# nordmtr/quantpy

Hardware: AMD Instinct MI355X
Metric: state reconstructions/sec (3-qubit MLE) (higher is better)
Workload: dtype f64

## Files before the change

### quantpy_amd/csrc/qt_small.h

```cpp
#pragma once
#include <hip/hip_runtime.h>
#include <stdint.h>

#include <type_traits>

#include "qt_linesearch.h"

namespace qt {

#ifdef QT_PHASE_TIMING
__device__ long long* g_qt_prof = nullptr;
#define QT_PROF_ROW \
  ((size_t)(blockIdx.x + threadIdx.y * gridDim.x) * (blockDim.x >> 6) + (threadIdx.x >> 6))
#define QT_STAMP(slot)                                                                                   \
  do {                                                                                                   \
    if (g_qt_prof && (threadIdx.x & 63) == 0)                                                            \
      g_qt_prof[QT_PROF_ROW * 32 + (slot)] = (long long)__builtin_readcyclecounter();                    \
  } while (0)
#define QT_STAMP_VAL(slot, val)                                                                          \
  do {                                                                                                   \
    if (g_qt_prof && (threadIdx.x & 63) == 0)                                                            \
      g_qt_prof[QT_PROF_ROW * 32 + (slot)] = (val);                                                      \
  } while (0)
#else
#define QT_STAMP(slot) do {} while (0)
#define QT_STAMP_VAL(slot, val) do {} while (0)
#endif

struct alignas(16) cd {
  double re, im;
};
__device__ __forceinline__ cd cmul(cd a, cd b) { return {a.re * b.re - a.im * b.im, a.re * b.im + a.im * b.re}; }
__device__ __forceinline__ cd cmulc(cd a, cd b) {
  return {a.re * b.re + a.im * b.im, a.im * b.re - a.re * b.im};
}
__device__ __forceinline__ cd cadd(cd a, cd b) { return {a.re + b.re, a.im + b.im}; }
__device__ __forceinline__ cd hs_term(cd a, cd b) {
  return {__builtin_fma(a.re, b.re, -(a.im * b.im)), __builtin_fma(a.re, b.im, a.im * b.re)};
}
__device__ __forceinline__ cd cscale(cd a, double s) { return {a.re * s, a.im * s}; }

__device__ __forceinline__ void wave_sync() {
  __builtin_amdgcn_wave_barrier();
  asm volatile("" ::: "memory");
}

template <int CTRL, int ROW_MASK = 0xf>
__device__ __forceinline__ double dpp_f64(double v) {
  const long long b = __builtin_bit_cast(long long, v);
  const int lo = __builtin_amdgcn_update_dpp(0, (int)(b & 0xffffffffLL), CTRL, ROW_MASK, 0xf, ROW_MASK == 0xf);
  const int hi = __builtin_amdgcn_update_dpp(0, (int)(b >> 32), CTRL, ROW_MASK, 0xf, ROW_MASK == 0xf);
  return __builtin_bit_cast(double, ((long long)hi << 32) | (unsigned int)lo);
}
__device__ __forceinline__ double readlane_f64(double v, int lane) {
  const long long b = __builtin_bit_cast(long long, v);
  const int lo = __builtin_amdgcn_readlane((int)(b & 0xffffffffLL), lane);
  const int hi = __builtin_amdgcn_readlane((int)(b >> 32), lane);
  return __builtin_bit_cast(double, ((long long)hi << 32) | (unsigned int)lo);
}
__device__ __forceinline__ double nanmax(double a, double b) { return (b > a || b != b) ? b : a; }

template <int G>
__device__ __forceinline__ double gsum(double v) {
  v += dpp_f64<0xB1>(v);
  v += dpp_f64<0x4E>(v);
  if (G >= 8) v += dpp_f64<0x141>(v);
  if (G >= 16) v += dpp_f64<0x140>(v);
  if (G == 64) {
    v += dpp_f64<0x142, 0xA>(v);
    v += dpp_f64<0x143, 0xC>(v);
    v = readlane_f64(v, 63);
  }
  return v;
}
template <int G>
__device__ __forceinline__ bool group_any(bool pred) {
  const unsigned long long votes = __builtin_amdgcn_ballot_w64(pred);
  if (G == 64) return votes != 0ull;
  const int lane = threadIdx.x & 63;
  return (votes & (((1ull << (G & 63)) - 1ull) << (lane / G * G))) != 0ull;
}
__device__ __forceinline__ double max_f64(double a, double b) {
  double r;
  asm("v_max_f64 %0, %1, %2" : "=v"(r) : "v"(a), "v"(b));
  return r;
}
template <int G>
__device__ __forceinline__ double gmax(double v) {
  const bool nan = group_any<G>(v != v);
  v = max_f64(v, dpp_f64<0xB1>(v));
  v = max_f64(v, dpp_f64<0x4E>(v));
  if (G >= 8) v = max_f64(v, dpp_f64<0x141>(v));
  if (G >= 16) v = max_f64(v, dpp_f64<0x140>(v));
  if (G == 64) {
    v = max_f64(v, dpp_f64<0x142, 0xA>(v));
    v = max_f64(v, dpp_f64<0x143, 0xC>(v));
    v = readlane_f64(v, 63);
  }
  return nan ? __builtin_nan("") : v;
}

__device__ __forceinline__ double recip_nr(double x) {
  double r = __builtin_amdgcn_rcp(x);
  r = fma(r, fma(-x, r, 1.0), r);
  return fma(r, fma(-x, r, 1.0), r);
}
__device__ __forceinline__ bool log_is_regular(double x) { return x > 0.0 && x < 1.7e308; }
__device__ __forceinline__ double fast_log(double x) {
  if (!(x > 0.0) || !(x < 1.7e308)) return x == 0.0 ? -__builtin_huge_val() : (x > 0.0 ? x : __builtin_nan(""));
  double m = __builtin_amdgcn_frexp_mant(x);
  int e = __builtin_amdgcn_frexp_exp(x);
  const bool low = m < 0.70710678118654752440;
  m = low ? m + m : m;
  e = low ? e - 1 : e;
  const double num = m - 1.0, den = m + 1.0;
  const double r = recip_nr(den);
  double sq = num * r;
  sq = fma(r, fma(-sq, den, num), sq);
  const double z = sq * sq;
  const double z2 = z * z, z4 = z2 * z2, z8 = z4 * z4;
  const double q0 = fma(z, 1.0 / 5.0, 1.0 / 3.0), q1 = fma(z, 1.0 / 9.0, 1.0 / 7.0);
  const double q2 = fma(z, 1.0 / 13.0, 1.0 / 11.0), q3 = fma(z, 1.0 / 17.0, 1.0 / 15.0);
  const double q4 = fma(z, 1.0 / 21.0, 1.0 / 19.0);
  const double r0 = fma(z2, q1, q0), r1 = fma(z2, q3, q2);
  const double pl = fma(z8, q4, fma(z4, r1, r0));
  const double lm = fma(sq + sq, pl * z, sq + sq);
  const double ed = (double)e;
  return fma(ed, 6.93147180369123816490e-01, fma(ed, 1.90821492927058770002e-10, lm));
}

constexpr bool kLiftSingleNegative = true;

__device__ __forceinline__ double fast_rsqrt(double x) {
  double y = __builtin_amdgcn_rsq(x);
  double e = fma(-x * y, y, 1.0);
  y = fma(y * e, fma(e, 0.375, 0.5), y);
  e = fma(-x * y, y, 1.0);
  return fma(y * e, 0.5, y);
}

template <int UNR>
__device__ __forceinline__ void dot_block(const double* __restrict__ base, size_t stride, unsigned lane_off,
                                          const double* lds_vec, int m, double (&acc)[4]) {
  double av[UNR];
#pragma unroll
  for (int u = 0; u < UNR; ++u) av[u] = base[(size_t)(m + u) * stride + lane_off];
#pragma unroll
  for (int u = 0; u < UNR; ++u) acc[u & 3] = fma(av[u], lds_vec[m + u], acc[u & 3]);
  __builtin_amdgcn_sched_group_barrier(0x020, UNR, 0);
#pragma unroll
  for (int u = 0; u < UNR; u += 4) {
    __builtin_amdgcn_sched_group_barrier(0x100, 2, 0);
    __builtin_amdgcn_sched_group_barrier(0x002, 4, 0);
  }
}
template <int UNR>
__device__ __forceinline__ double dot_global(const double* __restrict__ base, size_t stride, unsigned lane_off,
                                             const double* lds_vec, int n) {
  double acc[4] = {0.0, 0.0, 0.0, 0.0};
  int m = 0;
  for (; m + UNR <= n; m += UNR) dot_block<UNR>(base, stride, lane_off, lds_vec, m, acc);
  if (UNR > 8 && m + 8 <= n) {
    dot_block<8>(base, stride, lane_off, lds_vec, m, acc);
    m += 8;
  }
  if (UNR > 4 && m + 4 <= n) {
    dot_block<4>(base, stride, lane_off, lds_vec, m, acc);
    m += 4;
  }
  for (; m < n; ++m) acc[0] = fma(base[(size_t)m * stride + lane_off], lds_vec[m], acc[0]);
  return (acc[0] + acc[1]) + (acc[2] + acc[3]);
}

__device__ __forceinline__ void rotation(double app, double aqq, cd apq, double& cs, cd& w) {
  const double ab2 = apq.re * apq.re + apq.im * apq.im;
  cs = 1.0;
  w = cd{0.0, 0.0};
  if (ab2 > 1e-300) {
    const double dl = 0.5 * (aqq - app);
    const double x = fma(dl, dl, ab2);
    double y = __builtin_amdgcn_rsq(x);
    y = fma(y * fma(-x * y, y, 1.0), 0.5, y);
    const double den = fabs(dl) + x * y;
    double z = __builtin_amdgcn_rcp(den);
    z = fma(z, fma(-den, z, 1.0), z);
    const double u = copysign(z, dl);
    cs = fast_rsqrt(fma(u * u, ab2, 1.0));
    const double cu = cs * u;
    w = cd{cu * apq.re, cu * apq.im};
  }
}


struct ProductView {
  const double* T;
  const double* P1T;
  const double* wrowR;
  const int* rmap;
  const int* rinv;
  const int* fwd;
  const int* bwd;
  int R1;
  int uniform;
  double wuni;
  int enabled;
  int pairedT, pairedP;
  double cT[12], cP[12];
  const int* last;
};

struct PovmView {
  const double* Aw;
  const double* AwT;
  const double* PinvT;
  int M;
  ProductView pr;
  double jtol2 = 1e-28;
  const double* Ns = nullptr;
  int S = 0, K = 0;
  double ns_tot = 0.0;
  int extra = 0;
};

struct SpecArgs {
  const void* image;
  const double* Ns;
  double ns_tot, wuni, jtol2;
  int M, extra;
  double cT[12], cP[12];
};
template <bool GENERIC>
struct MleArgs {
  using type = PovmView;
};
template <>
struct MleArgs<false> {
  using type = SpecArgs;
};

__device__ __forceinline__ bool shots_match(double t_s, double total, double n_s, double ns_tot) {
  const double a = t_s * ns_tot, b = n_s * total;
  return fabs(a - b) <= 2e-15 * fabs(b);
}

__device__ __forceinline__ const double* centre_of(const double* centres, int G, int g0, int b, int dd) {
  return G > 1 ? centres + (size_t)((unsigned)(g0 + b) % (unsigned)G) * dd : centres;
}

struct EstOut {
// ... 435 lines not shown
  __device__ __forceinline__ static bool seg_check(const double (&dv)[4], const bool (&valid)[4], double total,
                                                   const Prefetch& pf, double ns_tot) {
    bool bad = false;
#pragma unroll
    for (int q = 0; q < 4; ++q) bad |= valid[q] & !shots_match(segsum_c<KK>(dv[q]), total, pf.ns[q], ns_tot);
    return bad;
  }
  __device__ static bool load_freq(const Ctx& c, const int64_t* counts, const Prefetch* pf = nullptr) {
    double part = 0.0;
    double* raw = c.rbuf();
    double* fq = c.freq();
    bool bad = false;
    double total, inv;
    if (pf && pf->ok) {
      double dv[4];
      bool valid[4];
#pragma unroll
      for (int q = 0; q < 4; ++q) {
        const int m = c.l + q * G;
        valid[q] = m < c.M;
        dv[q] = valid[q] ? (double)pf->v[q] : 0.0;
        raw[valid[q] ? m : c.Mp] = dv[q];
        part += dv[q];
      }
      total = gsum<G>(part);
      inv = 1.0 / total;
      if (pf->seg) {
        switch (c.pv.K) {
          case 2: bad = seg_check<2>(dv, valid, total, *pf, c.pv.ns_tot); break;
          case 4: bad = seg_check<4>(dv, valid, total, *pf, c.pv.ns_tot); break;
          case 8: bad = seg_check<8>(dv, valid, total, *pf, c.pv.ns_tot); break;
          default: bad = seg_check<16>(dv, valid, total, *pf, c.pv.ns_tot); break;
        }
      }
      wave_sync();
#pragma unroll
      for (int q = 0; q < 4; ++q) {
        const int m = c.l + q * G, mc = m < c.M ? m : c.M - 1;
        fq[mc] = raw[c.prod() ? c.trmap[mc] : mc] * inv;
      }
    } else {
      for (int m = c.l; m < c.M; m += G) {
        const double v = (double)counts[m];
        raw[m] = v;
        part += v;
      }
      total = gsum<G>(part);
      inv = 1.0 / total;
      wave_sync();
      if (c.prod()) {
        for (int m = c.l; m < c.M; m += G) fq[m] = raw[c.trmap[m]] * inv;
      } else {
        for (int m = c.l; m < c.M; m += G) fq[m] = raw[m] * inv;
      }
    }
    if (c.pv.Ns && !(pf && pf->seg)) {
      const int K = c.pv.K;
      for (int s = c.l; s < c.pv.S; s += G) {
        double t = 0.0;
        for (int k = 0; k < K; ++k) t += raw[s * K + k];
        const double ns = (pf && s == c.l) ? pf->ns[0] : c.pv.Ns[s];
        bad |= !shots_match(t, total, ns, c.pv.ns_tot);
      }
    }
    const unsigned long long votes = __builtin_amdgcn_ballot_w64(bad);
    const int lane = threadIdx.x & 63;
    const unsigned long long mine = (G == 64) ? ~0ull : (((1ull << (G & 63)) - 1ull) << (lane / G * G));
    wave_sync();
    return (votes & mine) == 0ull;
  }

  __device__ __forceinline__ static void prefetch_counts(Prefetch& pf, const int64_t* counts, const SpecArgs& a) {
    const int l = (threadIdx.x & 63) % G, M = a.M, nch = image_chunks(M), t = threadIdx.x;
    const uint4* img = reinterpret_cast<const uint4*>(a.image);
    const int* rinv = reinterpret_cast<const int*>(img + nch);
    pf.img = img[t < nch ? t : nch - 1];
    if constexpr (NQ == 3) pf.mat = MakeMatTab<true, D>::type::v[l];
    pf.ok = pf.seg = true;
#pragma unroll
    for (int q = 0; q < 4; ++q) {
      const int m = l + q * G, mc = m < M ? m : M - 1;
      pf.v[q] = counts[mc];
      pf.ri[q] = rinv[mc];
      pf.ns[q] = a.Ns[mc >> NQ];
    }
  }
  template <bool VCOEF = false, bool TWIN = false, int LT>
  __device__ static void make_ctx(CtxSV<LT>& c, double* smem_block, const SpecArgs& a, const Prefetch& pf,
                                  [[maybe_unused]] int twin = 0) {
    static_assert(VCOEF == (LT == 2), "the one-wave-per-SIMD kernels keep coefficients and lane tables in vector registers");
    const int lane = threadIdx.x & 63, wave = threadIdx.x >> 6;
    c.l = lane % G;
    const int slot = wave * TPW + lane / G;
    c.i = c.l / d;
    c.j = c.l % d;
    c.e = c.i * LD + c.j;
    c.M = a.M;
    c.Mp = (a.M + 1) & ~1;
    c.a = a;
    if (!(TWIN && twin) && (int)threadIdx.x < image_chunks(a.M)) reinterpret_cast<uint4*>(smem_block)[threadIdx.x] = pf.img;
    c.tfwd = reinterpret_cast<const int*>(smem_block);
    c.ttab = smem_block + image_last_ints(a.M) / 2;
    c.ptab = c.ttab + 24;
    c.sm = smem_block + table_doubles(a.M, 6) + slot * (trial_doubles(a.M, 6) + a.extra);
    if (TWIN && twin) c.sm = smem_block + twin_offset(a.M, 6, a.extra) + slot * trial_doubles(a.M, 6);
    if (c.l == 0) c.sm[oVec + D] = 0.0;
    __syncthreads();
    int xm = 0, zm = 0, ny = 0;
#pragma unroll
    for (int b = 0; b < NQ; ++b) {
      const int dig = (c.l >> (2 * b)) & 3;
      xm |= (dig == 1 || dig == 2) << b;
      zm |= (dig >= 2) << b;
      ny += dig == 2;
    }
    c.xm = xm;
    c.zm = zm;
    c.ny = ny & 3;
    param_owner(c.l, c.pi, c.pj, c.pkind);
    const int tt = (c.i * (c.i - 1)) / 2 + c.j;
    c.src_re = c.i == c.j ? c.i : c.i > c.j ? d + tt : D;
    c.src_im = c.i > c.j ? d + T + tt : D;
    const int sx = (c.i & 1) | ((c.i & 2) << 1) | ((c.i & 4) << 2), sz = (c.j & 1) | ((c.j & 2) << 1) | ((c.j & 4) << 2);
    c.bslot = sx ^ (3 * sz);
    if constexpr (NQ == 3 && LT != 0) {
      c.mpack[0] = (uint32_t)pf.mat;
      c.mpack[1] = (uint32_t)(pf.mat >> 32);
      if constexpr (VCOEF) {
#pragma unroll
        for (int s = 0; s < d; ++s) {
          const uint32_t e = (c.mpack[s / 4] >> (8 * (s % 4))) & 0xffu;
          c.mterm[s] = c.sm + oVec + (e & 63u);
          c.msign[s] = (e & 0x80u) << 24;
        }
        c.bflip[0] = (uint32_t)lane << 31;
        c.bflip[1] = ((uint32_t)lane << 30) & 0x80000000u;
        c.bflip[2] = ((uint32_t)lane << 29) & 0x80000000u;
        c.bflip[3] = ((uint32_t)__popc(c.i & c.j) << 30) & 0x80000000u;
      }
    }
#pragma unroll
    for (int k = 0; k < 12; ++k) {
      c.kT[k] = VCOEF ? pin_vgpr(a.cT[k]) : a.cT[k];
      c.kP[k] = VCOEF ? pin_vgpr(a.cP[k]) : a.cP[k];
    }
  }
  template <int KK>
  __device__ __forceinline__ static double gsum_above(double v) {
    if (KK < 2) v += dpp_f64<0xB1>(v);
    if (KK < 4) v += dpp_f64<0x4E>(v);
    if (G >= 8 && KK < 8) v += dpp_f64<0x141>(v);
    if (G >= 16 && KK < 16) v += dpp_f64<0x140>(v);
    if (G == 64) {
      v += dpp_f64<0x142, 0xA>(v);
      v += dpp_f64<0x143, 0xC>(v);
      v = readlane_f64(v, 63);
    }
    return v;
  }
  template <int LT>
  __device__ static bool load_freq(const CtxSV<LT>& c, const Prefetch& pf) {
    double dv[4], st[4];
    bool valid[4];
#pragma unroll
    for (int q = 0; q < 4; ++q) {
      valid[q] = c.l + q * G < c.M;
      dv[q] = valid[q] ? (double)pf.v[q] : 0.0;
      st[q] = segsum_c<d>(dv[q]);
    }
    const double total = gsum_above<d>((st[0] + st[1]) + (st[2] + st[3]));
    const double inv = 1.0 / total;
    bool bad = false;
#pragma unroll
    for (int q = 0; q < 4; ++q) bad |= valid[q] & !shots_match(st[q], total, pf.ns[q], c.a.ns_tot);
    double* fq = c.freq();
    double* dummy = c.rbuf();
#pragma unroll
    for (int q = 0; q < 4; ++q) *(valid[q] ? fq + pf.ri[q] : dummy) = dv[q] * inv;
    const unsigned long long votes = __builtin_amdgcn_ballot_w64(bad);
    const int lane = threadIdx.x & 63;
    const unsigned long long mine = (G == 64) ? ~0ull : (((1ull << (G & 63)) - 1ull) << (lane / G * G));
    wave_sync();
    return (votes & mine) == 0ull;
  }

  __device__ __forceinline__ static int ipow(int b, int e) {
    int r = 1;
    for (int q = 0; q < e; ++q) r *= b;
    return r;
  }
  template <bool FWD, int R1C = 0>
  __device__ __forceinline__ static double stage_value(const double* tb, int R1, int ent, int stride, const double* in) {
    const int base = ent & 0xffff, sel = ent >> 16;
    if (FWD) {
      const double* row = tb + sel * 4;
      return fma(row[3], in[base + 3 * stride],
                 fma(row[2], in[base + 2 * stride], fma(row[1], in[base + stride], row[0] * in[base])));
    }
    double acc = 0.0;
    if (R1C > 0) {
      double tv[R1C > 0 ? R1C : 1], iv[R1C > 0 ? R1C : 1];
#pragma unroll
      for (int t = 0; t < R1C; ++t) {
        tv[t] = tb[t * 4 + sel];
        iv[t] = in[base + t * stride];
      }
#pragma unroll
      for (int t = 0; t < R1C; ++t) acc = fma(tv[t], iv[t], acc);
      return acc;
    }
    for (int t = 0; t < R1; ++t) acc = fma(tb[t * 4 + sel], in[base + t * stride], acc);
    return acc;
  }
  template <bool FWD, int R1C, class C>
  __device__ __forceinline__ static void stage_run(const C& c, const double* tb, const int* tab, int n_out, int stride,
                                                   const double* in, double* out) {
    const int R1 = c.R1();
    for (int o = c.l; o < n_out; o += 2 * G) {
      const int o2 = o + G;
      const bool two = o2 < n_out;
      const int e0 = tab[o], e1 = tab[two ? o2 : o];
      const double v0 = stage_value<FWD, R1C>(tb, R1, e0, stride, in);
      const double v1 = stage_value<FWD, R1C>(tb, R1, e1, stride, in);
      out[o] = v0;
      if (two) out[o2] = v1;
    }
  }
  template <bool FWD, class C>
  __device__ static void stage(const C& c, const double* tb, const int* tab, int n_out, int stride, const double* in,
                               double* out) {
    if (FWD) stage_run<true, 0>(c, tb, tab, n_out, stride, in, out);
    else if (c.R1() == 6) stage_run<false, 6>(c, tb, tab, n_out, stride, in, out);
    else if (c.R1() == 4) stage_run<false, 4>(c, tb, tab, n_out, stride, in, out);
    else stage_run<false, 0>(c, tb, tab, n_out, stride, in, out);
    wave_sync();
  }
  template <int R1C, class C>
  __device__ __forceinline__ static double stage_last(const C& c, const double* tb, const int* tab, const double* in) {
    return stage_value<false, R1C>(tb, c.R1(), tab[c.l], 1 << (2 * (NQ - 1)), in);
  }
  __device__ __forceinline__ static int paired_bases(int q) { return ipow(6, q - 1) << (2 * (NQ - q)); }
  template <class C>
  __device__ __forceinline__ static void paired_forward(const C& c, int q, const double* in, double* out) {
    const int lk = 2 * (NQ - q), Kq = 1 << lk;
    if (c.l < paired_bases(q)) {
      const int rpre = c.l >> lk, krest = c.l & (Kq - 1);
      const double* ib = in + ((rpre * 4) << lk) + krest;
      double* ob = out + ((rpre * 6) << lk) + krest;
      const double x0 = ib[0];
      const double xa[3] = {ib[Kq], ib[2 * Kq], ib[3 * Kq]};
#pragma unroll
      for (int r = 0; r < 6; ++r) ob[r * Kq] = fma(c.cT(2 * r + 1), xa[r >> 1], c.cT(2 * r) * x0);
    }
    wave_sync();
  }
  template <bool PINV, class C>
  __device__ __forceinline__ static void paired_backward(const C& c, int q, const double* in, double* out) {
    const int lk = 2 * (NQ - q), Kq = 1 << lk;
    if (c.l < paired_bases(q)) {
      const int rpre = c.l >> lk, krest = c.l & (Kq - 1);
      const double* ib = in + ((rpre * 6) << lk) + krest;
      double* ob = out + ((rpre * 4) << lk) + krest;
      double y[6], acc = 0.0;
#pragma unroll
      for (int t = 0; t < 6; ++t) y[t] = ib[t * Kq];
#pragma unroll
      for (int t = 0; t < 6; ++t) acc = fma(PINV ? c.cP(2 * t) : c.cT(2 * t), y[t], acc);
      ob[0] = acc;
#pragma unroll
      for (int a = 0; a < 3; ++a) {
        const double v0 = PINV ? c.cP(4 * a + 1) : c.cT(4 * a + 1);
        const double v1 = PINV ? c.cP(4 * a + 3) : c.cT(4 * a + 3);
        ob[(a + 1) * Kq] = fma(v1, y[2 * a + 1], v0 * y[2 * a]);
      }
    }
    wave_sync();
  }

  template <bool PINV, class C>
  __device__ static double prod_backward(const C& c, const double* yn) {
    const double* tb = PINV ? c.tabP() : c.tabT();
    const double* in = yn;
    double* bufs[2] = {c.bufB(), c.rbuf()};
    int which = 0;
    if (PINV ? c.pairedP() : c.pairedT()) {
#pragma unroll
      for (int q = NQ; q >= 2; --q) {
        paired_backward<PINV>(c, q, in, bufs[which]);
        in = bufs[which];
        which ^= 1;
      }
      const int lk = 2 * (NQ - 1);
      return stage_value<false, 6>(tb, 6, (c.l & ((1 << lk) - 1)) | (c.l >> lk) << 16, 1 << lk, in);
    }
    if constexpr (C::kGeneric) {
      const int R1 = c.R1();
      const int* tab = c.tbwd;
#pragma unroll
      for (int q = NQ; q >= 2; --q) {
        const int stride = 1 << (2 * (NQ - q));
        const int n_out = ipow(R1, q - 1) * 4 * stride;
        stage<false>(c, tb, tab, n_out, stride, in, bufs[which]);
        tab += n_out;
        in = bufs[which];
        which ^= 1;
      }
      if (R1 == 6) return stage_last<6>(c, tb, tab, in);
      if (R1 == 4) return stage_last<4>(c, tb, tab, in);
// ... 310 lines not shown
      if (!(mag > 1e-13)) neg = neg > 0 ? 99 : neg;
      const double safe = mag > 1e-300 ? mag : 1e-300;
      if (k + 1 < d) {
        const double inv = recip_nr(safe);
        const double sinv = pos ? -inv : inv;
        const cd ajs{ajk.re * sinv, ajk.im * sinv};
        const bool upd = i > k && j > k;
        const double nre = fma(aik.re, ajs.re, fma(aik.im, ajs.im, a.re));
        const double nim = fma(aik.im, ajs.re, fma(-aik.re, ajs.im, a.im));
        a.re = upd ? nre : a.re;
        a.im = upd ? nim : a.im;
        A[c.e] = a;
        wave_sync();
      }
    }
    {
      const double dj = A[j * LD + j].re;
      const double mj = fabs(dj);
      const double rs = fast_rsqrt(mj > 1e-300 ? mj : 1e-300);
      if (i >= j) lmine = (i == j) ? cd{dj * rs, 0.0} : cd{a.re * rs, a.im * rs};
    }
    ok = neg == 0;
    if (neg_out) *neg_out = neg;
    if (kneg_out) *kneg_out = kneg;
    if (SPEC && spec_inv) *spec_inv = b;
    L[c.e] = lmine;
    wave_sync();
    const cd e = L[c.pi * LD + c.pj];
    const double x = c.pkind == 2 ? e.im : e.re;
    wave_sync();
    return x;
  }

  struct HelperLink {
    enum : int { kPending = 0, kGo = 1, kAbort = 2, kClaimed = 3, kRevoked = 4 };
    enum : int { kNothing = 0, kLifted = 1, kRefused = 2 };
    static constexpr int kHelperPolls = 1 << 15, kWaitPolls = 1 << 14, kClaimedPolls = 1 << 16;
    double* base;
    int pending;
    __device__ __forceinline__ static constexpr int doubles() { return MAT + D + 3; }
    __device__ __forceinline__ cd* result() const { return reinterpret_cast<cd*>(base); }
    __device__ __forceinline__ double* x() const { return base + MAT; }
    __device__ __forceinline__ int* verdict() const { return reinterpret_cast<int*>(base + MAT + D); }
    __device__ __forceinline__ int* lifted() const { return verdict() + 1; }
    __device__ __forceinline__ int* done() const { return verdict() + 2; }
    __device__ __forceinline__ int* gone() const { return verdict() + 3; }
    __device__ __forceinline__ int* ok() const { return verdict() + 4; }
    __device__ __forceinline__ static void publish(int* w, int v) {
      wave_sync();
      if ((threadIdx.x & 63) == 0) __hip_atomic_store(w, v, __ATOMIC_RELEASE, __HIP_MEMORY_SCOPE_WORKGROUP);
    }
    __device__ __forceinline__ static int peek(const int* w) {
      return __builtin_amdgcn_readfirstlane(__hip_atomic_load(w, __ATOMIC_RELAXED, __HIP_MEMORY_SCOPE_WORKGROUP));
    }
    __device__ __forceinline__ static bool claim(int* w, int from, int to) {
      int won = 0;
      if ((threadIdx.x & 63) == 0) {
        int expect = from;
        won = __hip_atomic_compare_exchange_strong(w, &expect, to, __ATOMIC_ACQ_REL, __ATOMIC_RELAXED,
                                                   __HIP_MEMORY_SCOPE_WORKGROUP);
      }
      return __builtin_amdgcn_readfirstlane(won) != 0;
    }
    template <int SLEEP>
    __device__ __forceinline__ static int poll(const int* w, int idle, int polls) {
      int v = idle;
#pragma unroll 1
      for (int n = 0; n < polls; ++n) {
        v = peek(w);
        if (v != idle) break;
        __builtin_amdgcn_s_sleep(SLEEP);
      }
      return v;
    }
    __device__ __forceinline__ void reset() {
      pending = 0;
      if ((threadIdx.x & 63) == 0) {
        *verdict() = kPending;
        *lifted() = kNothing;
        *done() = 0;
        *gone() = 0;
      }
    }
    __device__ __forceinline__ void decide(bool go) const { publish(verdict(), go ? kGo : kAbort); }
    __device__ __forceinline__ int await_lift(int e, cd& proj) {
      int v = poll<1>(lifted(), kNothing, kWaitPolls);
      if (v == kNothing) {
        if (claim(verdict(), kGo, kRevoked)) return kNothing;
        v = poll<1>(lifted(), kNothing, kClaimedPolls);
        if (v == kNothing) return kNothing;
      }
      __builtin_amdgcn_fence(__ATOMIC_ACQUIRE, "workgroup");
      if (v == kLifted) {
        proj = result()[e];
        pending = 1;
      }
      return v;
    }
    __device__ __forceinline__ bool collect(int l, double& xl, int& okl) const {
      if (poll<1>(done(), 0, kClaimedPolls) == 0) return false;
      __builtin_amdgcn_fence(__ATOMIC_ACQUIRE, "workgroup");
      xl = x()[l];
      okl = *ok();
      return true;
    }
    __device__ __forceinline__ void await_gone() const {
      poll<1>(gone(), 0, kClaimedPolls);
      __builtin_amdgcn_fence(__ATOMIC_ACQUIRE, "workgroup");
    }
  };
  struct CtxH {
    int l, i, j, e, pi, pj, pkind;
    cd *image, *second, *factor;
    const int* verdict;
    __device__ __forceinline__ cd* A() const { return image; }
    __device__ __forceinline__ cd* Bm() const { return factor; }
    __device__ __forceinline__ cd* V() const { return second; }
    __device__ __forceinline__ int verdict_load() const {
      return __hip_atomic_load(verdict, __ATOMIC_RELAXED, __HIP_MEMORY_SCOPE_WORKGROUP);
    }
    __device__ __forceinline__ static bool abandoned(int v) {
      v = __builtin_amdgcn_readfirstlane(v);
      return v != HelperLink::kPending && v != HelperLink::kGo;
    }
  };
  struct LateX {
    bool got;
    double x;
    int ok;
  };
  template <class Base>
  struct WithHelper : Base {
    HelperLink* link;
    LateX* late;
    double* xtra;
    __device__ __forceinline__ double* extra() const { return xtra; }
    static constexpr bool kHelper = true;
  };
  __device__ __forceinline__ static void param_owner(int l, int& pi, int& pj, int& pkind) {
    const bool diag = l < d, imag = l >= d + T;
    const int t = l - d - (imag ? T : 0);
    int ii = 1;
#pragma unroll
    for (int k = 2; k < d; ++k) ii += t >= (k * (k - 1)) / 2;
    pkind = diag ? 0 : imag ? 2 : 1;
    pi = diag ? l : ii;
    pj = diag ? l : t - (ii * (ii - 1)) / 2;
  }
  template <class C>
  __device__ static bool twin_lift(const C& t, const HelperLink& k, cd lin, cd& proj) {
    static_assert(G == 64, "one trial per wavefront");
    CtxH c = side_ctx(t, k, t.Bm());
    proj = cd{0.0, 0.0};
    const bool lifted = __builtin_amdgcn_readfirstlane((int)lift_single_negative(c, lin, d - 1, 1e-15, proj, nullptr)) != 0;
    QT_STAMP(6);
    if (HelperLink::template poll<1>(k.verdict(), HelperLink::kPending, HelperLink::kHelperPolls) != HelperLink::kGo) return false;
    QT_STAMP(7);
    if (!HelperLink::claim(k.verdict(), HelperLink::kGo, HelperLink::kClaimed)) return false;
    if (!lifted) {
      HelperLink::publish(k.lifted(), HelperLink::kRefused);
      return false;
    }
    k.result()[c.e] = proj;
    HelperLink::publish(k.lifted(), HelperLink::kLifted);
    return true;
  }
  template <class C>
  __device__ static void sweep_for(const C& t, const HelperLink& k, cd proj, cd* L) {
    CtxH c = side_ctx(t, k, L);
    int ok2;
    const double x2 = cholesky_param(c, proj, ok2);
    k.x()[c.l] = x2;
    if (c.l == 0) *k.ok() = ok2;
    HelperLink::publish(k.done(), 1);
    QT_STAMP(7);
  }
  template <class C>
  __device__ __forceinline__ static CtxH side_ctx(const C& t, const HelperLink& k, cd* L) {
    CtxH c;
    c.l = t.l;
    c.i = t.i;
    c.j = t.j;
    c.e = t.e;
    c.pi = t.pi;
    c.pj = t.pj;
    c.pkind = t.pkind;
    c.image = t.A();
    c.second = t.V();
    c.factor = L;
    c.verdict = k.verdict();
    return c;
  }

  template <class C>
  __device__ static bool lift_single_negative(const C& c, cd r, int kneg, double eps, cd& out,
                                              const cd* inverse = nullptr) {
    static_assert(G == 64, "one trial per wavefront: the flags below are wave-uniform");
    cd* Ai = c.A();
    cd* Vi = c.V();
    const int i = c.i, j = c.j;
    if (i == j) r.im = 0.0;
    cd b = r;
    if (inverse) b = *inverse;
#pragma unroll 1
    for (int s = inverse ? d : 0; s < d; ++s) {
      const int p = s < kneg ? s : (s < d - 1 ? s + 1 : kneg);
      Ai[c.e] = b;
      const double piv = readlane_f64(b.re, p * d + p);
      wave_sync();
      const cd bip = Ai[i * LD + p], bpj = Ai[p * LD + j];
      wave_sync();
      double inv = __builtin_amdgcn_rcp(piv);
      inv = fma(inv, fma(-piv, inv, 1.0), inv);
      inv = fma(inv, fma(-piv, inv, 1.0), inv);
      const cd t{bpj.re * inv, bpj.im * inv};
      const cd e = cmul(bip, t);
      cd nb{b.re - e.re, b.im - e.im};
      if (j == p) nb = cd{-bip.re * inv, -bip.im * inv};
      if (i == p) nb = (j == p) ? cd{inv, 0.0} : t;
      b = nb;
    }
    QT_STAMP(4);
    b = cscale(b, fast_rsqrt(gsum<G>(b.re * b.re + b.im * b.im)));
    bool certified = false, done = false;
#pragma unroll 1
    for (int k = 1; k <= 7 && !done; ++k) {
      Ai[c.e] = b;
      wave_sync();
      [[maybe_unused]] const int verdict = c.verdict_load();
      cd n{0.0, 0.0}, n2{0.0, 0.0};
#pragma unroll
      for (int q = 0; q < d; q += 2) {
        const cd u = Ai[i * LD + q], v = Ai[j * LD + q];
        n.re = fma(u.re, v.re, fma(u.im, v.im, n.re));
        n.im = fma(u.im, v.re, fma(-u.re, v.im, n.im));
        if (q + 1 < d) {
          const cd u2 = Ai[i * LD + q + 1], v2 = Ai[j * LD + q + 1];
          n2.re = fma(u2.re, v2.re, fma(u2.im, v2.im, n2.re));
          n2.im = fma(u2.im, v2.re, fma(-u2.re, v2.im, n2.im));
        }
      }
      n = cadd(n, n2);
      wave_sync();
      if (c.abandoned(verdict)) return false;
      const double pur = gsum<G>(n.re * n.re + n.im * n.im);
      b = cscale(n, fast_rsqrt(pur));
      const double defect = 1.0 - pur;
      QT_STAMP_VAL(20, k);
#ifdef QT_PHASE_TIMING
      if (k <= 5) QT_STAMP(25 + k);
#endif
      if (certified) done = true;
      else if (defect < 1e-7) certified = true;
      else if (k == 3 && !(defect < 0.05)) return false;
    }
    QT_STAMP(5);
    if (!done) return false;
    if (i == j) b.im = 0.0;
    b = cscale(b, 1.0 / gsum<G>(i == j ? b.re : 0.0));
    const double lam = gsum<G>(r.re * b.re + r.im * b.im);
    if (!(lam < eps)) return false;
    Ai[c.e] = r;
    Vi[c.e] = b;
    wave_sync();
    cd q{-lam * b.re, -lam * b.im};
#pragma unroll
    for (int k = 0; k < d; ++k) {
      const cd u = Ai[i * LD + k], v = Vi[j * LD + k];
      q.re = fma(u.re, v.re, fma(u.im, v.im, q.re));
      q.im = fma(u.im, v.re, fma(-u.re, v.im, q.im));
    }
    wave_sync();
    const double res2 = gsum<G>(q.re * q.re + q.im * q.im);
    const double nrm2 = gsum<G>(r.re * r.re + r.im * r.im);
    if (!(res2 <= 1e-26 * nrm2)) return false;
    const double w = eps - lam;
    cd o{fma(w, b.re, r.re), fma(w, b.im, r.im)};
    const double tr = gsum<G>(i == j ? o.re : 0.0);
    out = cd{o.re / tr, o.im / tr};
    return true;
  }

  template <bool SPEC = false, class C>
  __device__ static cd make_feasible(const C& c, cd r, double* xl, int* ok_out, double* lscale_out = nullptr) {
    int ok, neg, kneg;
    cd spec_inv{0.0, 0.0};
    double x = cholesky_param<SPEC && G == 64>(c, r, ok, &neg, &kneg, &spec_inv);
    QT_STAMP(3);
    cd out{0.0, 0.0};
    double lscale = 1.0;
    auto pd_epilogue = [&]() {
      const double tr = gsum<G>(c.i == c.j ? r.re : 0.0);
      out = cd{r.re / tr, r.im / tr};
      const double rst = tr > 0.0 ? fast_rsqrt(tr) : 1.0 / sqrt(tr);
      x = x * rst;
      lscale = rst;
    };
    const bool all_pd = __all(ok);
    [[maybe_unused]] bool go = false;
    if constexpr (C::kHelper) {
      go = kLiftSingleNegative && !all_pd && __builtin_amdgcn_readfirstlane(neg) == 1 &&
           __builtin_amdgcn_readfirstlane(kneg) == d - 1;
      c.link->decide(go);
    }
    if (G < 64 || all_pd || (!xl && lscale_out)) pd_epilogue();
    if (!all_pd) {
      cd proj;
      bool lifted = false;
      [[maybe_unused]] bool refused = false;
      if constexpr (C::kHelper) {
        if (go) {
          const int came = c.link->await_lift(c.e, proj);
          QT_STAMP(31);
          if (came == HelperLink::kLifted) {
            QT_STAMP(6);
            if (lscale_out) *lscale_out = 1.0;
            return proj;
          }
          refused = came == HelperLink::kRefused;
        }
      }
      if constexpr (G == 64) {
        if (kLiftSingleNegative && !refused && __builtin_amdgcn_readfirstlane(neg) == 1) {
          const int kn = __builtin_amdgcn_readfirstlane(kneg);
          lifted = __builtin_amdgcn_readfirstlane(
                       (int)lift_single_negative(c, r, kn, 1e-15, proj, SPEC && kn == d - 1 ? &spec_inv : nullptr)) != 0;
        }
      }
      if (!lifted) proj = psd_project(c, r, 1e-15);
      QT_STAMP(6);
      int ok2 = 1;
      double x2 = xl ? cholesky_param(c, proj, ok2) : 0.0;
      if (lifted && xl && !__all(ok2 || ok)) {
        proj = psd_project(c, r, 1e-15);
        x2 = cholesky_param(c, proj, ok2);
      }
      QT_STAMP(7);
      if (xl) lscale = 1.0;
      if (!ok) {
        out = proj;
        x = x2;
        ok = ok2;
      }
    }
    if (xl) *xl = x;
    if (ok_out) *ok_out = ok;
    if (lscale_out) *lscale_out = lscale;
    return out;
  }

  template <class C>
  __device__ static cd build_llh(const C& c, double xl, double& tr) {
    double* vx = c.vec();
    cd* L = c.Bm();
    vx[c.l] = xl;
    tr = gsum<G>(xl * xl);
    wave_sync();
    const int i = c.i, j = c.j;
    L[c.e] = cd{vx[c.src_re], vx[c.src_im]};
    wave_sync();
    cd m{0.0, 0.0};
#pragma unroll
    for (int k = 0; k < d; ++k) {
      const cd u = L[i * LD + k], v = L[j * LD + k];
      m.re = fma(u.re, v.re, fma(u.im, v.im, m.re));
      m.im = fma(u.im, v.re, fma(-u.re, v.im, m.im));
    }
    return m;
  }

  struct StartPoint {
    cd rho;
    double lscale;
  };
  template <bool DEFER = false, class C, bool LATE = false>
  __device__ static void nll_grad(const C& c, double xl, double& f, double& gl, cd* rho_l = nullptr,
                                  bool want_grad = true, const StartPoint* start = nullptr, DeferredValue* dv = nullptr) {
    static_assert(!DEFER || !C::kGeneric, "the deferred value needs the compile-time row count of the specialised shape");
    double tr;
    QT_STAMP(11);
    cd m;
    if constexpr (LATE) {
      m = start->rho;
    } else if (start) {
      tr = gsum<G>(xl * xl);
      m = cd{start->rho.re * tr, start->rho.im * tr};
    } else {
      m = build_llh(c, xl, tr);
    }
    QT_STAMP(12);
    cd* A = c.A();
    const cd rho_e = start ? start->rho : cd{m.re / tr, m.im / tr};
    if (rho_l) *rho_l = rho_e;
    A[c.e] = rho_e;
    wave_sync();
    const double bl = bloch_of(c, A);
    QT_STAMP(13);
    double* vec = c.vec();
    vec[c.l] = bl;
    wave_sync();
    double fpart = 0.0;
    const double* fr = c.freq();
    double* rb = c.rbuf();
    double wl;
    if (c.prod()) {
      const int R1 = c.R1();
      const bool paired = c.pairedT() != 0;
      const int* tab = c.tfwd;
      const double* in = vec;
#pragma unroll
      for (int q = 1; q < NQ; ++q) {
        const int stride = 1 << (2 * (NQ - q));
        const int n_out = ipow(R1, q) * stride;
        double* out = ((NQ - 1 - q) & 1) ? rb : c.bufB();
        if (paired) {
          paired_forward(c, q, in, out);
        } else if constexpr (C::kGeneric) {
          stage<true>(c, c.tabT(), tab, n_out, stride, in, out);
          tab += n_out;
        }
        in = out;
      }
      QT_STAMP(14);
      if constexpr (DEFER) {
        stage_n_log<true, true, true>(c, tab, in, fr, rb, dv);
      } else if constexpr (!C::kGeneric) {
        fpart = stage_n_log<true, true>(c, tab, in, fr, rb);
      } else {
        if (!paired) fpart = stage_n_log<false, false>(c, tab, in, fr, rb);
        else if (c.uniform()) fpart = stage_n_log<true, true>(c, tab, in, fr, rb);
        else fpart = stage_n_log<true, false>(c, tab, in, fr, rb);
      }
      if constexpr (!DEFER) f = -gsum<G>(fpart);
      wave_sync();
      QT_STAMP(15);
      if (!want_grad) return;
      wl = prod_backward<false>(c, rb);
      QT_STAMP(16);
    } else if constexpr (C::kGeneric) {
      for (int m0 = 0; m0 < c.M; m0 += G) {
        const int mm = m0 + c.l;
        if (mm < c.M) {
          const double pe = row_dot(c, c.pv.AwT, mm, vec) * d + 1e-10;
          fpart += fr[mm] * fast_log(pe);
          rb[mm] = fr[mm] * recip_nr(pe);
// ... 754 lines not shown
```

Baseline: 110.7 million.

## Trim wavefront reductions, add diagonal trace reduction, unroll natural-order pivot elimination

Wave-level sum and max reductions drop the row masks on the final two DPP row-broadcast steps, since only lane 63 is read afterwards. A specialised gtrace reduction sums only the 8 diagonal lanes of the 8x8 matrix using one DPP shift and a few readlanes instead of a full tree, and it replaces every trace computation. The helper-side lift uses a compile-time natural pivot order with a fully unrolled elimination loop. The power-iteration loop folds its exit conditions into one branch and checks abandonment without an early return. The risks are subtle lane-index assumptions in gtrace (lane i*9 holds diagonal entry i for d=8) and a longer loop iteration when the work is abandoned.

```diff
diff --git a/quantpy_amd/csrc/qt_small.h b/quantpy_amd/csrc/qt_small.h
--- a/quantpy_amd/csrc/qt_small.h
+++ b/quantpy_amd/csrc/qt_small.h
@@ -67,11 +67,21 @@
   if (G >= 8) v += dpp_f64<0x141>(v);
   if (G >= 16) v += dpp_f64<0x140>(v);
   if (G == 64) {
-    v += dpp_f64<0x142, 0xA>(v);
-    v += dpp_f64<0x143, 0xC>(v);
+    v += dpp_f64<0x142>(v);
+    v += dpp_f64<0x143>(v);
     v = readlane_f64(v, 63);
   }
   return v;
+}
+template <int G>
+__device__ __forceinline__ double gtrace(bool diag, double x) {
+  double v = diag ? x : 0.0;
+  if (G != 64) return gsum<G>(v);
+  v += 0.0;
+  v += dpp_f64<0x119>(v);
+  const double hi = v + readlane_f64(v, 45);
+  const double lo = v + readlane_f64(v, 9);
+  return readlane_f64(hi + readlane_f64(lo, 27), 63);
 }
 template <int G>
 __device__ __forceinline__ bool group_any(bool pred) {
@@ -93,8 +103,8 @@
   if (G >= 8) v = max_f64(v, dpp_f64<0x141>(v));
   if (G >= 16) v = max_f64(v, dpp_f64<0x140>(v));
   if (G == 64) {
-    v = max_f64(v, dpp_f64<0x142, 0xA>(v));
-    v = max_f64(v, dpp_f64<0x143, 0xC>(v));
+    v = max_f64(v, dpp_f64<0x142>(v));
+    v = max_f64(v, dpp_f64<0x143>(v));
     v = readlane_f64(v, 63);
   }
   return nan ? __builtin_nan("") : v;
@@ -836,8 +846,8 @@
     if (G >= 8 && KK < 8) v += dpp_f64<0x141>(v);
     if (G >= 16 && KK < 16) v += dpp_f64<0x140>(v);
     if (G == 64) {
-      v += dpp_f64<0x142, 0xA>(v);
-      v += dpp_f64<0x143, 0xC>(v);
+      v += dpp_f64<0x142>(v);
+      v += dpp_f64<0x143>(v);
       v = readlane_f64(v, 63);
     }
     return v;
@@ -1454,7 +1464,7 @@
     static_assert(G == 64, "one trial per wavefront");
     CtxH c = side_ctx(t, k, t.Bm());
     proj = cd{0.0, 0.0};
-    const bool lifted = __builtin_amdgcn_readfirstlane((int)lift_single_negative(c, lin, d - 1, 1e-15, proj, nullptr)) != 0;
+    const bool lifted = __builtin_amdgcn_readfirstlane((int)lift_single_negative<true>(c, lin, d - 1, 1e-15, proj, nullptr)) != 0;
     QT_STAMP(6);
     if (HelperLink::template poll<1>(k.verdict(), HelperLink::kPending, HelperLink::kHelperPolls) != HelperLink::kGo) return false;
     QT_STAMP(7);
@@ -1494,7 +1504,7 @@
     return c;
   }
 
-  template <class C>
+  template <bool NATURAL = false, class C>
   __device__ static bool lift_single_negative(const C& c, cd r, int kneg, double eps, cd& out,
                                               const cd* inverse = nullptr) {
     static_assert(G == 64, "one trial per wavefront: the flags below are wave-uniform");
@@ -1504,9 +1514,7 @@
     if (i == j) r.im = 0.0;
     cd b = r;
     if (inverse) b = *inverse;
-#pragma unroll 1
-    for (int s = inverse ? d : 0; s < d; ++s) {
-      const int p = s < kneg ? s : (s < d - 1 ? s + 1 : kneg);
+    auto eliminate = [&](int p) {
       Ai[c.e] = b;
       const double piv = readlane_f64(b.re, p * d + p);
       wave_sync();
@@ -1521,12 +1529,21 @@
       if (j == p) nb = cd{-bip.re * inv, -bip.im * inv};
       if (i == p) nb = (j == p) ? cd{inv, 0.0} : t;
       b = nb;
+    };
+    if constexpr (NATURAL) {
+      if (!inverse) {
+#pragma unroll
+        for (int p = 0; p < d; ++p) eliminate(p);
+      }
+    } else {
+#pragma unroll 1
+      for (int s = inverse ? d : 0; s < d; ++s) eliminate(s < kneg ? s : (s < d - 1 ? s + 1 : kneg));
     }
     QT_STAMP(4);
     b = cscale(b, fast_rsqrt(gsum<G>(b.re * b.re + b.im * b.im)));
-    bool certified = false, done = false;
+    bool certified = false, called_off = false;
 #pragma unroll 1
-    for (int k = 1; k <= 7 && !done; ++k) {
+    for (int k = 1;; ++k) {
       Ai[c.e] = b;
       wave_sync();
       [[maybe_unused]] const int verdict = c.verdict_load();
@@ -1544,7 +1561,7 @@
       }
       n = cadd(n, n2);
       wave_sync();
-      if (c.abandoned(verdict)) return false;
+      called_off = c.abandoned(verdict);
       const double pur = gsum<G>(n.re * n.re + n.im * n.im);
       b = cscale(n, fast_rsqrt(pur));
       const double defect = 1.0 - pur;
@@ -1552,14 +1569,13 @@
 #ifdef QT_PHASE_TIMING
       if (k <= 5) QT_STAMP(25 + k);
 #endif
-      if (certified) done = true;
-      else if (defect < 1e-7) certified = true;
-      else if (k == 3 && !(defect < 0.05)) return false;
+      if (called_off | certified | (k == 7) | ((k == 3) & !(defect < 0.05))) break;
+      certified = defect < 1e-7;
     }
     QT_STAMP(5);
-    if (!done) return false;
+    if (called_off || !certified) return false;
     if (i == j) b.im = 0.0;
-    b = cscale(b, 1.0 / gsum<G>(i == j ? b.re : 0.0));
+    b = cscale(b, 1.0 / gtrace<G>(i == j, b.re));
     const double lam = gsum<G>(r.re * b.re + r.im * b.im);
     if (!(lam < eps)) return false;
     Ai[c.e] = r;
@@ -1578,7 +1594,7 @@
     if (!(res2 <= 1e-26 * nrm2)) return false;
     const double w = eps - lam;
     cd o{fma(w, b.re, r.re), fma(w, b.im, r.im)};
-    const double tr = gsum<G>(i == j ? o.re : 0.0);
+    const double tr = gtrace<G>(i == j, o.re);
     out = cd{o.re / tr, o.im / tr};
     return true;
   }
@@ -1592,7 +1608,7 @@
     cd out{0.0, 0.0};
     double lscale = 1.0;
     auto pd_epilogue = [&]() {
-      const double tr = gsum<G>(c.i == c.j ? r.re : 0.0);
+      const double tr = gtrace<G>(c.i == c.j, r.re);
       out = cd{r.re / tr, r.im / tr};
       const double rst = tr > 0.0 ? fast_rsqrt(tr) : 1.0 / sqrt(tr);
       x = x * rst;
```

Result: faster. 113.2 million, median of 6 (+2.2%).
